# aponte411/minGPT-distributed

Measured on AMD Instinct MI355X. Metric: tokens/sec (whole node), GPT-2 124M seq1024 bf16, higher is better.
Workload: dtype bf16; 1 GPU; model=gpt2, global_batch=128, seq_len=1024, parallelism=dp1, micro_batch_per_gpu=128, hip_graph=False

## Files before the change

csrc/bindings.cpp:

```cpp
#include <torch/extension.h>
#include <ATen/hip/impl/HIPGuardImplMasqueradingAsCUDA.h>
#include <ATen/hip/impl/HIPStreamMasqueradingAsCUDA.h>

#include "comm.h"
#include "kernels.h"

namespace {

using mg::bf16_t;

hipStream_t cur_stream() { return c10::hip::getCurrentHIPStreamMasqueradingAsCUDA().stream(); }
using DevGuard = c10::hip::HIPGuardMasqueradingAsCUDA;

#define CHECK_DEV(t) TORCH_CHECK((t).is_cuda(), #t " must be a GPU tensor")
#define CHECK_CONTIG(t) TORCH_CHECK((t).is_contiguous(), #t " must be contiguous")
#define CHECK_BF16(t) \
  CHECK_DEV(t);       \
  TORCH_CHECK((t).scalar_type() == at::kBFloat16, #t " must be bf16")
#define CHECK_F32(t) \
  CHECK_DEV(t);      \
  TORCH_CHECK((t).scalar_type() == at::kFloat, #t " must be fp32")
#define CHECK_I64(t) \
  CHECK_DEV(t);      \
  TORCH_CHECK((t).scalar_type() == at::kLong, #t " must be int64")
// ... 82 lines not shown
  }
  const unsigned long long* ap = nullptr;
  int groups = 0;
  int64_t* seqp = nullptr;
  long seq_ld = 0;
  if (am_part.has_value()) {
    TORCH_CHECK(pd && am_part->scalar_type() == at::kLong && am_part->is_contiguous() && am_part->dim() == 2 &&
                am_part->size(0) == B, "embedding_fwd: am_part int64 [B, G] with pos_dev");
    ap = reinterpret_cast<const unsigned long long*>(am_part->data_ptr<int64_t>());
    groups = (int)am_part->size(1);
    if (seq.has_value()) {
      TORCH_CHECK(seq->scalar_type() == at::kLong && seq->is_contiguous() && seq->dim() == 2 && seq->size(0) == B,
                  "embedding_fwd: seq int64 [B, L]");
      seqp = seq->data_ptr<int64_t>();
      seq_ld = seq->size(1);
    }
  }
  DevGuard g(idx.device());
  auto out = at::empty({B, T, D}, wte.options());
  mg::embedding_fwd(idx.data_ptr<int64_t>(), bp(wte), bp(wpe), bp(out), (int)(B * T), (int)T,
                    (int)D, (int)wte.size(0), (float)p, (uint64_t)seed, cur_stream(), pd, ap, groups,
                    ap ? idx.data_ptr<int64_t>() : nullptr, seqp, seq_ld, (int)pos_stride, (int)wpe.size(0));
  return out;
}

void embedding_bwd(const at::Tensor& idx, const at::Tensor& dout,
                   const c10::optional<at::Tensor>& dwte, const c10::optional<at::Tensor>& dwpe,
                   double p, int64_t seed) {
  CHECK_I64(idx); CHECK_BF16(dout); CHECK_CONTIG(dout); CHECK_CONTIG(idx);
  const int64_t B = idx.size(0), T = idx.size(1), D = dout.size(-1);
  TORCH_CHECK(dout.numel() == B * T * D, "embedding_bwd: shape mismatch");
  if (dwte.has_value()) { CHECK_F32(*dwte); TORCH_CHECK(dwte->size(-1) == D); }
  if (dwpe.has_value()) { CHECK_F32(*dwpe); TORCH_CHECK(dwpe->size(-1) == D && dwpe->size(0) >= T); }
  DevGuard g(idx.device());
  mg::embedding_bwd(idx.data_ptr<int64_t>(), bp(dout), fp_opt(dwte), fp_opt(dwpe), (int)(B * T),
                    (int)T, (int)D, dwte.has_value() ? (int)(dwte->numel() / D) : 0, (float)p, (uint64_t)seed, cur_stream());
}

std::vector<at::Tensor> xent_fwd(const at::Tensor& logits, const at::Tensor& targets, int64_t V) {
  CHECK_BF16(logits); CHECK_I64(targets); CHECK_CONTIG(logits); CHECK_CONTIG(targets);
  const int64_t ld = logits.size(-1), M = logits.numel() / ld;
  TORCH_CHECK(targets.numel() == M && V <= ld && ld % 8 == 0, "xent: shape mismatch");
  DevGuard g(logits.device());
  auto opts = logits.options().dtype(at::kFloat);
  auto loss_row = at::empty({M}, opts);
  auto lse = at::empty({M}, opts);
  auto out = at::empty({2}, opts);
  mg::xent_fwd(bp(logits), targets.data_ptr<int64_t>(), fp(loss_row), fp(lse), fp(out), (int)M,
               (int)V, (int)ld, cur_stream());
  return {out, lse};
}

at::Tensor xent_bwd(const at::Tensor& logits, const at::Tensor& targets, const at::Tensor& lse,
                    const at::Tensor& gscale, const at::Tensor& out, int64_t V) {
  CHECK_BF16(logits); CHECK_I64(targets); CHECK_F32(lse); CHECK_F32(gscale); CHECK_F32(out);
  const int64_t ld = logits.size(-1), M = logits.numel() / ld;
  TORCH_CHECK(targets.numel() == M && lse.numel() == M, "xent_bwd: shape mismatch");
  DevGuard g(logits.device());
  auto dl = at::empty_like(logits);
  mg::xent_bwd(bp(logits), targets.data_ptr<int64_t>(), fp(lse), fp(gscale), fp(out) + 1, bp(dl),
               (int)M, (int)V, (int)ld, cur_stream());
  return dl;
}

std::vector<at::Tensor> xent_fused(const at::Tensor& logits, const at::Tensor& targets, int64_t V) {
  CHECK_BF16(logits); CHECK_I64(targets); CHECK_CONTIG(logits); CHECK_CONTIG(targets);
  const int64_t ld = logits.size(-1), M = logits.numel() / ld;
  TORCH_CHECK(targets.numel() == M && V <= ld && ld % 8 == 0, "xent_fused: shape mismatch");
  if (mg::xent_fused_nv((int)ld) == 0) return {};
  DevGuard g(logits.device());
  auto opts = logits.options().dtype(at::kFloat);
  auto loss_row = at::empty({M}, opts);
  auto out = at::empty({2}, opts);
  auto dl = at::empty_like(logits);
  mg::xent_fused(bp(logits), targets.data_ptr<int64_t>(), fp(loss_row), fp(out), bp(dl), (int)M,
                 (int)V, (int)ld, cur_stream());
  return {out, dl};
}

void xent_scale_(const at::Tensor& dlogits, const at::Tensor& gscale) {
  CHECK_BF16(dlogits); CHECK_CONTIG(dlogits); CHECK_F32(gscale);
  TORCH_CHECK(dlogits.numel() % 8 == 0, "xent_scale_: numel must be a multiple of 8");
  DevGuard g(dlogits.device());
  mg::xent_scale(bp(dlogits), fp(gscale), dlogits.numel(), cur_stream());
}

void set_graph_state(const c10::optional<at::Tensor>& seed_ofs, const c10::optional<at::Tensor>& opt_hp) {
  if (seed_ofs.has_value()) {
    TORCH_CHECK(seed_ofs->scalar_type() == at::kLong && seed_ofs->is_cuda() && seed_ofs->numel() >= 1);
  }
  if (opt_hp.has_value()) { CHECK_F32(*opt_hp); TORCH_CHECK(opt_hp->numel() >= 2); }
  mg::set_graph_state(seed_ofs.has_value() ? reinterpret_cast<const uint64_t*>(seed_ofs->data_ptr<int64_t>()) : nullptr,
                      opt_hp.has_value() ? fp(*opt_hp) : nullptr);
}

void grad_sumsq(const at::Tensor& grad, double grad_scale, const at::Tensor& out) {
  CHECK_F32(grad); CHECK_F32(out); CHECK_CONTIG(grad);
  TORCH_CHECK(out.numel() >= 2);
  DevGuard g(grad.device());
  auto ws = at::empty({(int64_t)(mg::grad_norm_workspace() / 4)}, grad.options());
  mg::grad_sumsq(fp(grad), grad.numel(), (float)grad_scale, fp(ws), fp(out), cur_stream());
}

void grad_sumsq_chunks(const at::Tensor& chunk_start, const at::Tensor& chunk_len,
                       const at::Tensor& grad, double grad_scale, const at::Tensor& out,
                       int64_t table_end) {
  CHECK_I64(chunk_start); CHECK_DEV(chunk_len); CHECK_CONTIG(grad); CHECK_F32(out);
  TORCH_CHECK(chunk_len.scalar_type() == at::kInt, "chunk_len must be int32");
// ... 112 lines not shown
at::Tensor transpose(const at::Tensor& src, int64_t ldd) {
  CHECK_BF16(src); CHECK_CONTIG(src);
  TORCH_CHECK(src.dim() == 2, "transpose: 2-D input");
  const int64_t R = src.size(0), C = src.size(1);
  if (ldd <= 0) ldd = R;
  TORCH_CHECK(ldd >= R, "transpose: ldd < rows");
  DevGuard g(src.device());
  auto dst = at::empty({C, ldd}, src.options());
  mg::transpose(bp(src), bp(dst), (int)R, (int)C, (int)ldd, cur_stream());
  return dst;
}

at::Tensor dropout_bwd(const at::Tensor& dy, double p, int64_t seed) {
  CHECK_BF16(dy); CHECK_CONTIG(dy);
  const int64_t N = dy.size(-1), M = dy.numel() / N;
  TORCH_CHECK(N % 8 == 0, "dropout_bwd: last dim must be a multiple of 8");
  DevGuard g(dy.device());
  auto dx = at::empty_like(dy);
  mg::dropout_bwd(bp(dy), bp(dx), M, (int)N, (float)p, (uint64_t)seed, cur_stream());
  return dx;
}

at::Tensor dropout_bias_grad(const at::Tensor& dy, const at::Tensor& db, double p, int64_t seed) {
  CHECK_BF16(dy); CHECK_F32(db); CHECK_CONTIG(dy);
  const int64_t N = dy.size(-1), M = dy.numel() / N;
  TORCH_CHECK(N % 8 == 0 && db.numel() == N, "dropout_bias_grad: shape mismatch");
  DevGuard g(dy.device());
  auto dx = at::empty_like(dy);
  mg::dropout_bias_grad(bp(dy), bp(dx), fp(db), M, (int)N, (float)p, (uint64_t)seed, cur_stream());
  return dx;
}

void bias_grad(const at::Tensor& dy, const at::Tensor& db) {
  CHECK_BF16(dy); CHECK_F32(db); CHECK_CONTIG(dy);
  const int64_t N = dy.size(-1), M = dy.numel() / N;
  TORCH_CHECK(N % 8 == 0 && db.numel() == N, "bias_grad: shape mismatch");
  DevGuard g(dy.device());
  mg::bias_grad(bp(dy), fp(db), M, (int)N, cur_stream());
}

void gemm(const at::Tensor& a, const at::Tensor& b, const at::Tensor& c, int64_t layout, int64_t epi,
          const c10::optional<at::Tensor>& bias, const c10::optional<at::Tensor>& aux,
          const c10::optional<at::Tensor>& resid, double p, int64_t seed, int64_t M, int64_t N,
          const c10::optional<at::Tensor>& dbias) {
  CHECK_BF16(a); CHECK_BF16(b); CHECK_DEV(c);
  CHECK_CONTIG(a); CHECK_CONTIG(b); CHECK_CONTIG(c);
  TORCH_CHECK(a.dim() == 2 && b.dim() == 2 && c.dim() == 2, "gemm: 2-D operands required");
  TORCH_CHECK(layout >= 0 && layout <= 2 && epi >= 0 && epi <= 7 && epi != 5, "gemm: bad layout/epilogue");
  TORCH_CHECK((epi != 6 || layout == 0) && (epi != 7 || layout == 1), "gemm: fragment-ordered GELU' epilogues: 6 NT, 7 NN");
  const int64_t lda = a.size(1), ldb = b.size(1), ldc = c.size(1);
  TORCH_CHECK(lda % 8 == 0 && ldb % 8 == 0 && ldc % 8 == 0, "gemm: row strides must be multiples of 8");
  TORCH_CHECK(M > 0 && N > 0 && M <= c.size(0) && N <= ldc, "gemm: output bounds");
  int64_t K, a_ext, b_ext, ka, kb;
  if (layout == 0) {
    K = lda; ka = lda; kb = ldb; a_ext = a.size(0); b_ext = b.size(0);
    TORCH_CHECK(lda == ldb, "gemm NT: K mismatch");
    TORCH_CHECK(M <= a_ext && N <= (epi == 0 ? ldc : b_ext), "gemm NT: shape mismatch");
    TORCH_CHECK(c.scalar_type() == at::kBFloat16, "gemm NT: bf16 output");
  } else if (layout == 1) {
    K = lda; ka = lda; kb = b.size(0); a_ext = a.size(0); b_ext = ldb;
    TORCH_CHECK(kb <= K && M <= a_ext && N <= ldb && (epi == 0 || epi == 4 || epi == 7), "gemm NN: shape mismatch");
    TORCH_CHECK(c.scalar_type() == at::kBFloat16, "gemm NN: bf16 output");
  } else {
    K = a.size(0); ka = K; kb = b.size(0); a_ext = lda; b_ext = ldb;
    TORCH_CHECK(kb == K && M <= lda && N <= ldb && epi == 0, "gemm TN: shape mismatch");
    TORCH_CHECK(c.scalar_type() == at::kFloat, "gemm TN: fp32 accumulate output");
  }
  TORCH_CHECK(K % 8 == 0, "gemm: K must be a multiple of 8");
  const bf16_t* bias_p = nullptr;
  if (bias.has_value() && bias->defined()) {
    CHECK_BF16(*bias);
// ... 720 lines not shown
```

csrc/include/kernels.h:

```cpp
#pragma once
#include <hip/hip_runtime.h>
#include <stddef.h>
#include <stdint.h>

namespace mg {
typedef uint16_t bf16_t;

void layernorm_fwd(const bf16_t* x, const bf16_t* w, const bf16_t* b, bf16_t* y, float* mean,
                   float* rstd, int M, int D, float eps, hipStream_t stream);
void layernorm_bwd(const bf16_t* dy, const bf16_t* x, const bf16_t* w, const float* mean,
                   const float* rstd, const bf16_t* dres, bf16_t* dx, float* dw, float* db,
                   float* workspace, int M, int D, hipStream_t stream, bf16_t* dz = nullptr,
                   float* dzb = nullptr, float p = 0.f, uint64_t seed = 0);
size_t layernorm_bwd_workspace(int M, int D, bool drop);
int ln_bwd_grid(int M, int D, bool drop);

void embedding_fwd(const int64_t* idx, const bf16_t* wte, const bf16_t* wpe, bf16_t* out, int M,
                   int T, int D, int V, float p, uint64_t seed, hipStream_t stream,
                   const int* pos_dev = nullptr,
                   const unsigned long long* am_part = nullptr,
                   int am_groups = 0,
                   int64_t* tok = nullptr,
                   int64_t* seq = nullptr,
                   long seq_ld = 0,
                   int pos_stride = 0,
                   int pos_rows = 0);
unsigned int debug_error_bits();
void embedding_bwd(const int64_t* idx, const bf16_t* dout, float* dwte, float* dwpe, int M, int T,
                   int D, int V, float p, uint64_t seed, hipStream_t stream);

void xent_fwd(const bf16_t* logits, const int64_t* targets, float* loss_row, float* lse, float* out,
              int M, int V, int ld, hipStream_t stream);
void xent_bwd(const bf16_t* logits, const int64_t* targets, const float* lse, const float* gscale,
              const float* inv_n, bf16_t* dlogits, int M, int V, int ld, hipStream_t stream);
int xent_fused_nv(int ld);
void xent_fused(const bf16_t* logits, const int64_t* targets, float* loss_row, float* out,
                bf16_t* dlogits, int M, int V, int ld, hipStream_t stream);
void xent_scale(bf16_t* dlogits, const float* gscale, long n, hipStream_t stream);

void set_graph_state(const uint64_t* seed_ofs, const float* opt_hp);
const uint64_t* graph_seed_ofs();
const float* graph_opt_hp();
size_t grad_norm_workspace();
void grad_sumsq(const float* grad, long n, float grad_scale, float* workspace, float* out,
                hipStream_t stream);
void grad_sumsq_chunks(const int64_t* chunk_start, const int* chunk_len, int n_chunks,
                       const void* grad, bool grad_bf16, float grad_scale, float* workspace,
                       float* out, hipStream_t stream);
void adamw_step(const int64_t* chunk_start, const int* chunk_len, const float* chunk_wd,
                const int64_t* moment_start, int n_chunks, float* master, bf16_t* param,
                const void* grad, bool grad_bf16, float* m, float* v, const float* norm, float lr,
                float b1, float b2, float eps, int step, float grad_scale, float clip,
                hipStream_t stream, float* zero_grad = nullptr);
void f32_to_bf16(const float* src, bf16_t* dst, long n, hipStream_t stream);
void comm_proxy(const void* src, void* dst, long n16, long total16, int channels, double gbps,
                hipStream_t stream);

constexpr int kGemvSegK = 4096;
bool gemv_supported(int B, int K);
struct GemvArgmax {
  unsigned long long* part;
  int* pos;
};
int gemv_grid(int N, int B);
void gemv(const bf16_t* x, const bf16_t* W, bf16_t* y, int B, int N, int K, long ldy, const bf16_t* bias,
          const bf16_t* resid, int epi, hipStream_t stream, const bf16_t* lnw = nullptr,
          const bf16_t* lnb = nullptr, float eps = 1e-5f, const GemvArgmax* am = nullptr);
bool gemv_nt_weights();
bool gemv_w8_supported(int B, int K);
// ... 86 lines not shown
```

csrc/kernels/elementwise.hip:

```cpp
#include "common.h"
#include "kernels.h"

using namespace mg;

namespace {

constexpr int kGrid = 4096;

__global__ __launch_bounds__(256) void bias_act_kernel(const bf16_t* __restrict__ x,
                                                       const bf16_t* __restrict__ b,
                                                       bf16_t* __restrict__ pre,
                                                       bf16_t* __restrict__ y, long n8, int N,
                                                       int act) {
  for (long i = (long)blockIdx.x * 256 + threadIdx.x; i < n8; i += (long)gridDim.x * 256) {
    const long e = i * 8;
    const int c = (int)(e % N);
    float v[8], bb[8];
    unpack8(ld16(x + e), v);
    if (b) {
      unpack8(ld16(b + c), bb);
#pragma unroll
      for (int j = 0; j < 8; ++j) v[j] += bb[j];
    }
    if (act == 1) {
// ... 65 lines not shown
                                                                bf16_t* __restrict__ dx,
                                                                float* __restrict__ db, int M, int N,
                                                                uint64_t seed, uint32_t thr,
                                                                float scale, const uint64_t* sofs) {
  constexpr int RG = 256 / CVB;
  __shared__ __attribute__((aligned(16))) float red[RG][CVB * 8];
  seed = eff_seed(seed, sofs);
  const int cv = threadIdx.x % CVB, rg = threadIdx.x / CVB;
  const int c = (blockIdx.x * CVB + cv) * 8;
  float s[8] = {0, 0, 0, 0, 0, 0, 0, 0};
  if (c < N) {
    for (long r = (long)blockIdx.y * RG + rg; r < M; r += (long)gridDim.y * RG) {
      float g[8];
      const long e = r * N + c;
      unpack8(ld16(dy + e), g);
      rowdrop8(g, seed, r, c, N, thr, scale);
      st16(dx + e, pack8(g));
#pragma unroll
      for (int j = 0; j < 8; ++j) s[j] += g[j];
    }
  }
#pragma unroll
  for (int j = 0; j < 8; ++j) red[rg][cv * 8 + j] = s[j];
  __syncthreads();
  for (int k = threadIdx.x; k < CVB * 8; k += 256) {
    const int col = blockIdx.x * CVB * 8 + k;
    float t = 0.f;
#pragma unroll
    for (int i = 0; i < RG; ++i) t += red[i][k];
    if (col < N) atomicAdd(db + col, t);
  }
}

template <int CVB>
__global__ __launch_bounds__(256) void bias_grad_kernel(const bf16_t* __restrict__ dy,
                                                        float* __restrict__ db, int M, int N, long ld) {
  constexpr int RG = 256 / CVB;
  __shared__ __attribute__((aligned(16))) float red[RG][CVB * 8];
  const int cv = threadIdx.x % CVB, rg = threadIdx.x / CVB;
  const int c = (blockIdx.x * CVB + cv) * 8;
  float s[8] = {0, 0, 0, 0, 0, 0, 0, 0};
  if (c < N) {
    for (long r = (long)blockIdx.y * RG + rg; r < M; r += (long)gridDim.y * RG) {
      float g[8];
      unpack8(ld16(dy + r * ld + c), g);
#pragma unroll
      for (int j = 0; j < 8; ++j) s[j] += g[j];
    }
  }
#pragma unroll
  for (int j = 0; j < 8; ++j) red[rg][cv * 8 + j] = s[j];
  __syncthreads();
  for (int k = threadIdx.x; k < CVB * 8; k += 256) {
    const int col = blockIdx.x * CVB * 8 + k;
    float t = 0.f;
#pragma unroll
    for (int i = 0; i < RG; ++i) t += red[i][k];
    if (col < N) atomicAdd(db + col, t);
  }
}

__global__ __launch_bounds__(256) void transpose_kernel(const bf16_t* __restrict__ src,
                                                        bf16_t* __restrict__ dst, int R, int C,
                                                        int ldd) {
  __shared__ uint4 t[16 * 8 * 16];
  const int r0 = blockIdx.y * 128, c0 = blockIdx.x * 128;
  {
    const int rb = threadIdx.x >> 4, cb = threadIdx.x & 15;
    uint32_t w[8][4];
#pragma unroll
    for (int i = 0; i < 8; ++i) {
      const int r = r0 + 8 * rb + i, c = c0 + 8 * cb;
      uint4 v = make_uint4(0, 0, 0, 0);
      if (r < R) {
        if (c + 8 <= C) {
          v = ld16(src + (long)r * C + c);
        } else if (c < C) {
          alignas(16) bf16_t e[8] = {0, 0, 0, 0, 0, 0, 0, 0};
          for (int q = 0; q < 8 && c + q < C; ++q) e[q] = src[(long)r * C + c + q];
          v = *reinterpret_cast<const uint4*>(e);
// ... 61 lines not shown
                                                       graph_seed_ofs());
}

static int bias_cvb(int N) { return ((N / 8) % 64 != 0 && (N / 8) % 32 == 0) ? 32 : 64; }

static dim3 bias_grid(long M, int N, int cvb) {
  const int cx = cdiv(N, cvb * 8);
  int ry = (int)std::max<long>(1, std::min<long>(512, M / 64));
  while (cx * ry > 2048 && ry > 1) ry >>= 1;
  return dim3(cx, ry);
}

void dropout_bias_grad(const bf16_t* dy, bf16_t* dx, float* db, long M, int N, float p, uint64_t seed,
                       hipStream_t stream) {
  const uint32_t thr = dropout_threshold16(p);
  const int cvb = bias_cvb(N);
  const dim3 grid = bias_grid(M, N, cvb);
  if (cvb == 32)
    dropout_bias_grad_kernel<32><<<grid, 256, 0, stream>>>(dy, dx, db, (int)M, N, seed, thr,
                                                           dropout_scale16(thr), graph_seed_ofs());
  else
    dropout_bias_grad_kernel<64><<<grid, 256, 0, stream>>>(dy, dx, db, (int)M, N, seed, thr,
                                                           dropout_scale16(thr), graph_seed_ofs());
}

void transpose(const bf16_t* src, bf16_t* dst, int R, int C, int ldd, hipStream_t stream) {
  transpose_kernel<<<dim3(cdiv(C, 128), cdiv(ldd, 128)), 256, 0, stream>>>(src, dst, R, C, ldd);
}

void bias_grad(const bf16_t* dy, float* db, long M, int N, hipStream_t stream, long ld) {
  const int cvb = bias_cvb(N);
  const dim3 grid = bias_grid(M, N, cvb);
  if (ld <= 0) ld = N;
  if (cvb == 32)
    bias_grad_kernel<32><<<grid, 256, 0, stream>>>(dy, db, (int)M, N, ld);
  else
    bias_grad_kernel<64><<<grid, 256, 0, stream>>>(dy, db, (int)M, N, ld);
}

}
```

csrc/kernels/embedding.hip:

```cpp
#include "common.h"
#include "kernels.h"

using namespace mg;

namespace {

__global__ __launch_bounds__(256) void emb_fwd_kernel(const int64_t* __restrict__ idx,
                                                      const bf16_t* __restrict__ wte,
                                                      const bf16_t* __restrict__ wpe,
                                                      bf16_t* __restrict__ out, int M, int T, int D, int V,
                                                      unsigned int* __restrict__ err,
                                                      uint64_t seed, uint32_t thr, float scale,
                                                      int use_dropout, const uint64_t* sofs,
                                                      const int* __restrict__ pos_dev, int pos_stride,
                                                      int pos_rows,
                                                      const unsigned long long* __restrict__ am_part,
                                                      int am_groups, int64_t* __restrict__ tok_out,
                                                      int64_t* __restrict__ seq, long seq_ld) {
  const int lane = threadIdx.x & 63;
  const long m = (long)blockIdx.x * 4 + (threadIdx.x >> 6);
  if (m >= M) return;
  seed = eff_seed(seed, sofs);
  long tok;
  if (am_part) {
    unsigned long long best = 0;
    for (int i = lane; i < am_groups; i += 64) {
      const unsigned long long k = am_part[m * am_groups + i];
      best = k > best ? k : best;
    }
#pragma unroll
    for (int o = 32; o > 0; o >>= 1) {
      const unsigned lo = __shfl_xor((unsigned)best, o, 64), hi = __shfl_xor((unsigned)(best >> 32), o, 64);
      const unsigned long long k = ((unsigned long long)hi << 32) | lo;
      best = k > best ? k : best;
    }
    tok = amax_index(best);
    if (lane == 0) {
      if (tok_out) tok_out[m] = tok;
      if (seq) seq[m * seq_ld + *pos_dev] = tok;
    }
  } else {
    tok = idx[m];
  }
  MG_CHECK_INDEX(tok, tok >= 0 && tok < V, 0, err, 1u)
  int t = pos_dev ? *pos_dev : (int)(m % T);
  if (pos_dev && pos_stride) t = min(max(pos_dev[m * pos_stride], 0), pos_rows - 1);
  for (int c = lane * 8; c < D; c += 512) {
    float a[8], p[8];
    unpack8(ld16(wte + tok * D + c), a);
    unpack8(ld16(wpe + (long)t * D + c), p);
#pragma unroll
    for (int j = 0; j < 8; ++j) a[j] += p[j];
    if (use_dropout) rowdrop8(a, seed, m, c, D, thr, scale);
    st16(out + m * D + c, pack8(a));
  }
}

__global__ __launch_bounds__(256) void emb_bwd_wte_kernel(const int64_t* __restrict__ idx,
                                                          const bf16_t* __restrict__ dout,
                                                          float* __restrict__ dwte, int M, int D, int V,
                                                          unsigned int* __restrict__ err,
                                                          uint64_t seed, uint32_t thr, float scale,
                                                          int use_dropout, const uint64_t* sofs) {
  const int lane = threadIdx.x & 63;
  const long m = (long)blockIdx.x * 4 + (threadIdx.x >> 6);
  if (m >= M) return;
  seed = eff_seed(seed, sofs);
  long tok = idx[m];
  MG_CHECK_INDEX(tok, tok >= 0 && tok < V, 0, err, 2u)
  for (int c0 = 0; c0 < D; c0 += 512) {
    const int c = c0 + lane * 8;
    float g[8];
    if (c < D) {
      unpack8(ld16(dout + m * D + c), g);
      if (use_dropout) rowdrop8(g, seed, m, c, D, thr, scale);
    }
#pragma unroll
    for (int k = 0; k < 8; ++k) {
      const int src = 8 * k + (lane >> 3);
      float val = 0.f;
#pragma unroll
      for (int j = 0; j < 8; ++j) {
        const float t = __shfl(g[j], src, 64);
        if ((lane & 7) == j) val = t;
      }
      const int col = c0 + 64 * k + lane;
      if (col < D) atomicAdd(dwte + tok * D + col, val);
    }
  }
}

__global__ __launch_bounds__(64) void emb_bwd_wpe_kernel(const bf16_t* __restrict__ dout,
                                                         float* __restrict__ dwpe, int B, int T, int D,
                                                         uint64_t seed, uint32_t thr, float scale,
                                                         int use_dropout, const uint64_t* sofs) {
  const int t = blockIdx.x;
  const int c = blockIdx.y * 512 + threadIdx.x * 8;
  if (c >= D) return;
  seed = eff_seed(seed, sofs);
  float s[8] = {0, 0, 0, 0, 0, 0, 0, 0};
  for (int b = 0; b < B; ++b) {
    const long m = (long)b * T + t;
    float g[8];
    unpack8(ld16(dout + m * D + c), g);
    if (use_dropout) rowdrop8(g, seed, m, c, D, thr, scale);
#pragma unroll
    for (int j = 0; j < 8; ++j) s[j] += g[j];
  }
  float* dst = dwpe + (long)t * D + c;
#pragma unroll
  for (int j = 0; j < 8; ++j) dst[j] += s[j];
}

}

namespace mg {

void embedding_fwd(const int64_t* idx, const bf16_t* wte, const bf16_t* wpe, bf16_t* out, int M,
                   int T, int D, int V, float p, uint64_t seed, hipStream_t stream, const int* pos_dev,
                   const unsigned long long* am_part, int am_groups, int64_t* tok, int64_t* seq,
                   long seq_ld, int pos_stride, int pos_rows) {
  const uint32_t thr = dropout_threshold16(p);
  emb_fwd_kernel<<<cdiv(M, 4), 256, 0, stream>>>(idx, wte, wpe, out, M, T, D, V, debug_err_word(), seed, thr,
                                                 dropout_scale16(thr), p > 0.f,
                                                 graph_seed_ofs(), pos_dev, pos_stride, pos_rows, am_part,
                                                 am_groups, tok, seq, seq_ld);
}

void embedding_bwd(const int64_t* idx, const bf16_t* dout, float* dwte, float* dwpe, int M, int T,
                   int D, int V, float p, uint64_t seed, hipStream_t stream) {
  const uint32_t thr = dropout_threshold16(p);
  const float scale = dropout_scale16(thr);
  if (dwte)
    emb_bwd_wte_kernel<<<cdiv(M, 4), 256, 0, stream>>>(idx, dout, dwte, M, D, V, debug_err_word(), seed, thr, scale,
                                                       p > 0.f, graph_seed_ofs());
  if (dwpe) {
    dim3 grid(T, cdiv(D, 512));
    emb_bwd_wpe_kernel<<<grid, 64, 0, stream>>>(dout, dwpe, M / T, T, D, seed, thr, scale, p > 0.f,
                                                graph_seed_ofs());
  }
}

unsigned int* debug_err_word() {
#ifdef MG_DEBUG
  static unsigned int* w = nullptr;
  if (!w) {
    (void)hipMalloc(&w, sizeof(unsigned int));
    (void)hipMemset(w, 0, sizeof(unsigned int));
  }
  return w;
#else
  return nullptr;
#endif
}

unsigned int debug_error_bits() {
#ifdef MG_DEBUG
  unsigned int v = 0u;
  (void)hipDeviceSynchronize();
  (void)hipMemcpy(&v, debug_err_word(), sizeof(v), hipMemcpyDeviceToHost);
  (void)hipMemset(debug_err_word(), 0, sizeof(v));
  (void)hipDeviceSynchronize();
  return v;
#else
  return 0u;
#endif
}

}
```

csrc/kernels/xent.hip:

```cpp
#include "common.h"
#include "kernels.h"

using namespace mg;

namespace {

__global__ __launch_bounds__(256) void xent_fwd_kernel(const bf16_t* __restrict__ logits,
                                                       const int64_t* __restrict__ targets,
                                                       float* __restrict__ loss_row,
                                                       float* __restrict__ lse_out, int V, int ld,
                                                       unsigned int* __restrict__ err) {
  __shared__ float red[8];
  const long row = blockIdx.x;
  const bf16_t* lr = logits + row * ld;
  float mx = -INFINITY, sm = 0.f;
  const int V8 = V & ~7;
  for (int c = threadIdx.x * 8; c < V8; c += 256 * 8) {
    float v[8];
    unpack8(ld16(lr + c), v);
    float lm = v[0];
#pragma unroll
    for (int j = 1; j < 8; ++j) lm = fmaxf(lm, v[j]);
    if (lm > mx) {
      sm *= __expf(mx - lm);
      mx = lm;
    }
#pragma unroll
    for (int j = 0; j < 8; ++j) sm += __expf(v[j] - mx);
  }
  for (int c = V8 + threadIdx.x; c < V; c += 256) {
    const float v = bf2f(lr[c]);
    if (v > mx) {
      sm *= __expf(mx - v);
      mx = v;
    }
    sm += __expf(v - mx);
  }
  const float gmx = block_max<4>(mx, red);
  sm = (mx == -INFINITY) ? 0.f : sm * __expf(mx - gmx);
  const float gsm = block_sum<4>(sm, red + 4);
  if (threadIdx.x == 0) {
    const float lse = gmx + __logf(gsm);
    lse_out[row] = lse;
    long t = targets[row];
  MG_CHECK_INDEX(t, t < V, -1, err, 4u)
    loss_row[row] = (t < 0) ? 0.f : lse - bf2f(lr[t]);
  }
}

__global__ __launch_bounds__(1024) void xent_finalize_kernel(const float* __restrict__ loss_row,
                                                             const int64_t* __restrict__ targets,
                                                             float* __restrict__ out, int M) {
  __shared__ float red[32];
  float s = 0.f, n = 0.f;
  for (int i = threadIdx.x; i < M; i += 1024) {
    s += loss_row[i];
    n += targets[i] >= 0 ? 1.f : 0.f;
  }
  s = block_sum<16>(s, red);
  n = block_sum<16>(n, red + 16);
  if (threadIdx.x == 0) {
    const float inv = n > 0.f ? 1.f / n : 0.f;
    out[0] = s * inv;
    out[1] = inv;
  }
}

__global__ __launch_bounds__(256) void xent_bwd_kernel(const bf16_t* __restrict__ logits,
                                                       const int64_t* __restrict__ targets,
                                                       const float* __restrict__ lse,
                                                       const float* __restrict__ gscale,
                                                       const float* __restrict__ inv_n,
                                                       bf16_t* __restrict__ dlogits, int V, int ld,
                                                       unsigned int* __restrict__ err) {
  const long row = blockIdx.x;
  long t = targets[row];
  MG_CHECK_INDEX(t, t < V, -1, err, 4u)
  const float g = (t < 0) ? 0.f : gscale[0] * inv_n[0];
  const float l = lse[row];
  const bf16_t* lr = logits + row * ld;
  bf16_t* dr = dlogits + row * ld;
  for (int c = threadIdx.x * 8; c < ld; c += 256 * 8) {
    float v[8];
    if (c + 8 <= V) {
      unpack8(ld16(lr + c), v);
#pragma unroll
      for (int j = 0; j < 8; ++j) v[j] = g * (__expf(v[j] - l) - ((c + j) == t ? 1.f : 0.f));
    } else {
#pragma unroll
      for (int j = 0; j < 8; ++j) {
        const int cj = c + j;
        v[j] = cj < V ? g * (__expf(bf2f(lr[cj]) - l) - (cj == t ? 1.f : 0.f)) : 0.f;
      }
    }
    st16(dr + c, pack8(v));
  }
}


__global__ __launch_bounds__(1024) void xent_count_kernel(const int64_t* __restrict__ targets,
                                                          float* __restrict__ out, int M) {
  __shared__ float red[16];
  float n = 0.f;
  for (int i = threadIdx.x; i < M; i += 1024) n += targets[i] >= 0 ? 1.f : 0.f;
  n = block_sum<16>(n, red);
  if (threadIdx.x == 0) out[1] = n > 0.f ? 1.f / n : 0.f;
}

template <int NV>
__global__ __launch_bounds__(1024) void xent_fused_kernel(const bf16_t* __restrict__ logits,
                                                          const int64_t* __restrict__ targets,
                                                          const float* __restrict__ inv_n,
                                                          float* __restrict__ loss_row,
                                                          bf16_t* __restrict__ dlogits, int V,
                                                          int ld, unsigned int* __restrict__ err) {
  __shared__ float red[32];
  const long row = blockIdx.x;
  const bf16_t* lr = logits + row * ld;
  bf16_t* dr = dlogits + row * ld;
  constexpr uint32_t NEG2 = 0xFF80FF80u;
  uint4 u[NV];
#pragma unroll
  for (int k = 0; k < NV; ++k) {
    const int c = (threadIdx.x + k * 1024) * 8;
    if (c + 8 <= V) {
      u[k] = ld16_nt(lr + c);
    } else if (c < V) {
      float f[8];
#pragma unroll
      for (int j = 0; j < 8; ++j) f[j] = (c + j < V) ? bf2f(lr[c + j]) : -INFINITY;
      u[k] = pack8(f);
    } else {
      u[k] = make_uint4(NEG2, NEG2, NEG2, NEG2);
    }
  }
  float mx = -INFINITY;
#pragma unroll
  for (int k = 0; k < NV; ++k) {
    float v[8];
    unpack8(u[k], v);
#pragma unroll
    for (int j = 0; j < 8; ++j) mx = fmaxf(mx, v[j]);
  }
  const float gmx = block_max<16>(mx, red);
#pragma unroll
  for (int k = 0; k < NV; ++k) reg_fence(u[k]);
  constexpr float L2E = 1.4426950408889634f;
  const float mb = gmx * L2E;
  float sm = 0.f;
#pragma unroll
  for (int k = 0; k < NV; ++k) {
    float v[8];
    unpack8(u[k], v);
#pragma unroll
    for (int j = 0; j < 8; ++j) sm += exp2f(fmaf(v[j], L2E, -mb));
  }
  const float gsm = block_sum<16>(sm, red + 16);
#pragma unroll
  for (int k = 0; k < NV; ++k) reg_fence(u[k]);
  const float lse = gmx + __logf(gsm);
  long t = targets[row];
  MG_CHECK_INDEX(t, t < V, -1, err, 4u)
  const float g = (t < 0) ? 0.f : inv_n[0];
  const float lb = lse * L2E;
#pragma unroll
  for (int k = 0; k < NV; ++k) {
    const int c = (threadIdx.x + k * 1024) * 8;
    if (c < ld) {
      float v[8];
      unpack8(u[k], v);
#pragma unroll
      for (int j = 0; j < 8; ++j) v[j] = g * (exp2f(fmaf(v[j], L2E, -lb)) - ((c + j) == t ? 1.f : 0.f));
      st16_nt(dr + c, pack8(v));
    }
  }
  if (threadIdx.x == 0) loss_row[row] = (t < 0) ? 0.f : lse - bf2f(lr[t]);
}

__global__ __launch_bounds__(256) void xent_scale_kernel(bf16_t* __restrict__ dl,
                                                         const float* __restrict__ gscale, long n8) {
  const float s = gscale[0];
  if (s == 1.f) return;
  for (long i = blockIdx.x * 256L + threadIdx.x; i < n8; i += (long)gridDim.x * 256) {
    float v[8];
    unpack8(ld16(dl + i * 8), v);
#pragma unroll
    for (int j = 0; j < 8; ++j) v[j] *= s;
    st16(dl + i * 8, pack8(v));
  }
}

}

namespace mg {

void xent_fwd(const bf16_t* logits, const int64_t* targets, float* loss_row, float* lse, float* out,
              int M, int V, int ld, hipStream_t stream) {
  xent_fwd_kernel<<<M, 256, 0, stream>>>(logits, targets, loss_row, lse, V, ld, debug_err_word());
  xent_finalize_kernel<<<1, 1024, 0, stream>>>(loss_row, targets, out, M);
}

void xent_bwd(const bf16_t* logits, const int64_t* targets, const float* lse, const float* gscale,
              const float* inv_n, bf16_t* dlogits, int M, int V, int ld, hipStream_t stream) {
  xent_bwd_kernel<<<M, 256, 0, stream>>>(logits, targets, lse, gscale, inv_n, dlogits, V, ld, debug_err_word());
}

}

namespace mg {

int xent_fused_nv(int ld) {
  const int nv = (ld / 8 + 1023) / 1024;
  return (nv >= 4 && nv <= 8) ? nv : 0;
}

void xent_fused(const bf16_t* logits, const int64_t* targets, float* loss_row, float* out,
                bf16_t* dlogits, int M, int V, int ld, hipStream_t stream) {
  xent_count_kernel<<<1, 1024, 0, stream>>>(targets, out, M);
  switch (xent_fused_nv(ld)) {
#define MG_XF(n) \
  case n: xent_fused_kernel<n><<<M, 1024, 0, stream>>>(logits, targets, out + 1, loss_row, dlogits, V, ld, debug_err_word()); break;
    MG_XF(4) MG_XF(5) MG_XF(6) MG_XF(7) MG_XF(8)
#undef MG_XF
    default: break;
  }
  xent_finalize_kernel<<<1, 1024, 0, stream>>>(loss_row, targets, out, M);
}

void xent_scale(bf16_t* dlogits, const float* gscale, long n, hipStream_t stream) {
  const long n8 = n / 8;
  const long blocks = std::min<long>((n8 + 255) / 256, 2048);
  xent_scale_kernel<<<(int)blocks, 256, 0, stream>>>(dlogits, gscale, n8);
}

}
```

Baseline: 1.147 million tokens/s.

## Sort tokens for embedding backward, parallelize xent reductions, unroll bias grad

Embedding wte backward now builds a token histogram, prefix scan and sorted order, then accumulates runs of equal tokens in registers. This replaces one atomic per row element with far fewer atomics. The wpe backward uses four waves per block with a shared-memory reduction. The cross-entropy count and finalize steps become a multi-block partial reduction plus a one-wave finalize instead of single-block kernels, and bias_grad gains multi-row unrolled loads for strided column slices. The cost is extra kernel launches and a zeroed workspace allocation on each call.

```diff
diff --git a/csrc/bindings.cpp b/csrc/bindings.cpp
--- a/csrc/bindings.cpp
+++ b/csrc/bindings.cpp
@@ -138,9 +138,14 @@
   TORCH_CHECK(dout.numel() == B * T * D, "embedding_bwd: shape mismatch");
   if (dwte.has_value()) { CHECK_F32(*dwte); TORCH_CHECK(dwte->size(-1) == D); }
   if (dwpe.has_value()) { CHECK_F32(*dwpe); TORCH_CHECK(dwpe->size(-1) == D && dwpe->size(0) >= T); }
+  TORCH_CHECK(D % 8 == 0 && (!fp_opt(dwte) || (uintptr_t)fp_opt(dwte) % 16 == 0),
+              "embedding_bwd: D must be a multiple of 8 and dwte 16-byte aligned");
   DevGuard g(idx.device());
-  mg::embedding_bwd(idx.data_ptr<int64_t>(), bp(dout), fp_opt(dwte), fp_opt(dwpe), (int)(B * T),
-                    (int)T, (int)D, dwte.has_value() ? (int)(dwte->numel() / D) : 0, (float)p, (uint64_t)seed, cur_stream());
+  const int64_t V = fp_opt(dwte) ? dwte->numel() / D : 0;
+  at::Tensor ws;
+  if (fp_opt(dwte)) ws = at::zeros({mg::embedding_bwd_workspace((int)(B * T), (int)V)}, idx.options().dtype(at::kInt));
+  mg::embedding_bwd(idx.data_ptr<int64_t>(), bp(dout), fp_opt(dwte), fp_opt(dwpe), ws.defined() ? ws.data_ptr<int>() : nullptr,
+                    (int)(B * T), (int)T, (int)D, (int)V, (float)p, (uint64_t)seed, cur_stream());
 }
 
 std::vector<at::Tensor> xent_fwd(const at::Tensor& logits, const at::Tensor& targets, int64_t V) {
@@ -152,7 +157,8 @@
   auto loss_row = at::empty({M}, opts);
   auto lse = at::empty({M}, opts);
   auto out = at::empty({2}, opts);
-  mg::xent_fwd(bp(logits), targets.data_ptr<int64_t>(), fp(loss_row), fp(lse), fp(out), (int)M,
+  auto ws = at::empty({mg::xent_scalar_workspace()}, opts);
+  mg::xent_fwd(bp(logits), targets.data_ptr<int64_t>(), fp(loss_row), fp(lse), fp(out), fp(ws), (int)M,
                (int)V, (int)ld, cur_stream());
   return {out, lse};
 }
@@ -179,7 +185,8 @@
   auto loss_row = at::empty({M}, opts);
   auto out = at::empty({2}, opts);
   auto dl = at::empty_like(logits);
-  mg::xent_fused(bp(logits), targets.data_ptr<int64_t>(), fp(loss_row), fp(out), bp(dl), (int)M,
+  auto ws = at::empty({mg::xent_scalar_workspace()}, opts);
+  mg::xent_fused(bp(logits), targets.data_ptr<int64_t>(), fp(loss_row), fp(out), fp(ws), bp(dl), (int)M,
                  (int)V, (int)ld, cur_stream());
   return {out, dl};
 }
@@ -358,11 +365,19 @@
 }
 
 void bias_grad(const at::Tensor& dy, const at::Tensor& db) {
-  CHECK_BF16(dy); CHECK_F32(db); CHECK_CONTIG(dy);
+  CHECK_BF16(dy); CHECK_F32(db);
+  const bool slice = dy.dim() == 2 && !dy.is_contiguous();
+  if (slice) {
+    TORCH_CHECK(dy.stride(1) == 1 && dy.stride(0) >= dy.size(1) && dy.stride(0) % 8 == 0 &&
+                (uintptr_t)dy.data_ptr() % 16 == 0, "bias_grad: a column slice needs unit column stride, "
+                "a row stride that is a multiple of 8 and a 16-byte aligned start");
+  } else {
+    CHECK_CONTIG(dy);
+  }
   const int64_t N = dy.size(-1), M = dy.numel() / N;
-  TORCH_CHECK(N % 8 == 0 && db.numel() == N, "bias_grad: shape mismatch");
+  TORCH_CHECK(N % 8 == 0 && db.numel() == N && db.is_contiguous(), "bias_grad: shape mismatch");
   DevGuard g(dy.device());
-  mg::bias_grad(bp(dy), fp(db), M, (int)N, cur_stream());
+  mg::bias_grad(bp(dy), fp(db), M, (int)N, cur_stream(), slice ? dy.stride(0) : 0);
 }
 
 void gemm(const at::Tensor& a, const at::Tensor& b, const at::Tensor& c, int64_t layout, int64_t epi,
diff --git a/csrc/include/kernels.h b/csrc/include/kernels.h
--- a/csrc/include/kernels.h
+++ b/csrc/include/kernels.h
@@ -26,15 +26,17 @@
                    int pos_stride = 0,
                    int pos_rows = 0);
 unsigned int debug_error_bits();
-void embedding_bwd(const int64_t* idx, const bf16_t* dout, float* dwte, float* dwpe, int M, int T,
+long embedding_bwd_workspace(int M, int V);
+void embedding_bwd(const int64_t* idx, const bf16_t* dout, float* dwte, float* dwpe, int* ws, int M, int T,
                    int D, int V, float p, uint64_t seed, hipStream_t stream);
 
+long xent_scalar_workspace();
 void xent_fwd(const bf16_t* logits, const int64_t* targets, float* loss_row, float* lse, float* out,
-              int M, int V, int ld, hipStream_t stream);
+              float* ws, int M, int V, int ld, hipStream_t stream);
 void xent_bwd(const bf16_t* logits, const int64_t* targets, const float* lse, const float* gscale,
               const float* inv_n, bf16_t* dlogits, int M, int V, int ld, hipStream_t stream);
 int xent_fused_nv(int ld);
-void xent_fused(const bf16_t* logits, const int64_t* targets, float* loss_row, float* out,
+void xent_fused(const bf16_t* logits, const int64_t* targets, float* loss_row, float* out, float* ws,
                 bf16_t* dlogits, int M, int V, int ld, hipStream_t stream);
 void xent_scale(bf16_t* dlogits, const float* gscale, long n, hipStream_t stream);
 
diff --git a/csrc/kernels/elementwise.hip b/csrc/kernels/elementwise.hip
--- a/csrc/kernels/elementwise.hip
+++ b/csrc/kernels/elementwise.hip
@@ -121,7 +121,9 @@
   }
 }
 
-template <int CVB>
+constexpr int kBiasRows = 4;
+
+template <int CVB, int ROWS>
 __global__ __launch_bounds__(256) void bias_grad_kernel(const bf16_t* __restrict__ dy,
                                                         float* __restrict__ db, int M, int N, long ld) {
   constexpr int RG = 256 / CVB;
@@ -130,11 +132,33 @@
   const int c = (blockIdx.x * CVB + cv) * 8;
   float s[8] = {0, 0, 0, 0, 0, 0, 0, 0};
   if (c < N) {
-    for (long r = (long)blockIdx.y * RG + rg; r < M; r += (long)gridDim.y * RG) {
-      float g[8];
-      unpack8(ld16(dy + r * ld + c), g);
-#pragma unroll
-      for (int j = 0; j < 8; ++j) s[j] += g[j];
+    float a[ROWS][8] = {};
+    const long step = (long)gridDim.y * RG;
+    for (long r = (long)blockIdx.y * RG + rg; r < M; r += ROWS * step) {
+      uint4 u[ROWS];
+#pragma unroll
+      for (int i = 0; i < ROWS; ++i) {
+        const long ri = r + i * step;
+        u[i] = ri < M ? ld16(dy + ri * ld + c) : make_uint4(0, 0, 0, 0);
+      }
+#pragma unroll
+      for (int i = 0; i < ROWS; ++i) {
+        float g[8];
+        unpack8(u[i], g);
+#pragma unroll
+        for (int j = 0; j < 8; ++j) a[i][j] += g[j];
+      }
+    }
+#pragma unroll
+    for (int j = 0; j < 8; ++j) {
+      float h[ROWS];
+#pragma unroll
+      for (int i = 0; i < ROWS; ++i) h[i] = a[i][j];
+#pragma unroll
+      for (int w = ROWS / 2; w > 0; w >>= 1)
+#pragma unroll
+        for (int i = 0; i < w; ++i) h[i] += h[i + w];
+      s[j] = h[0];
     }
   }
 #pragma unroll
@@ -262,10 +286,16 @@
   const int cvb = bias_cvb(N);
   const dim3 grid = bias_grid(M, N, cvb);
   if (ld <= 0) ld = N;
-  if (cvb == 32)
-    bias_grad_kernel<32><<<grid, 256, 0, stream>>>(dy, db, (int)M, N, ld);
-  else
-    bias_grad_kernel<64><<<grid, 256, 0, stream>>>(dy, db, (int)M, N, ld);
-}
-
-}
+  if (ld > N) {
+    if (cvb == 32)
+      bias_grad_kernel<32, kBiasRows><<<grid, 256, 0, stream>>>(dy, db, (int)M, N, ld);
+    else
+      bias_grad_kernel<64, kBiasRows><<<grid, 256, 0, stream>>>(dy, db, (int)M, N, ld);
+  } else if (cvb == 32) {
+    bias_grad_kernel<32, 1><<<grid, 256, 0, stream>>>(dy, db, (int)M, N, ld);
+  } else {
+    bias_grad_kernel<64, 1><<<grid, 256, 0, stream>>>(dy, db, (int)M, N, ld);
+  }
+}
+
+}
diff --git a/csrc/kernels/embedding.hip b/csrc/kernels/embedding.hip
--- a/csrc/kernels/embedding.hip
+++ b/csrc/kernels/embedding.hip
@@ -56,60 +56,219 @@
   }
 }
 
+
+constexpr int kCH = 32;
+
+MG_DEVICE void emb_wave_groups(int tok, bool valid, int lane, int& leader, int& rank, int& size) {
+  unsigned long long todo = __ballot(valid);
+  leader = lane, rank = 0, size = 0;
+  while (todo) {
+    const int l = __ffsll((long long)todo) - 1;
+    const int t = __shfl(tok, l, 64);
+    const unsigned long long same = __ballot(valid && tok == t);
+    if (valid && tok == t) {
+      leader = l;
+      rank = __popcll(same & ((1ull << lane) - 1ull));
+      size = __popcll(same);
+    }
+    todo &= ~same;
+  }
+}
+
+MG_DEVICE bool emb_token(const int64_t* __restrict__ idx, int m, int M, int V, unsigned int* err, int& tok) {
+  if (m >= M) return false;
+  long t = idx[m];
+  MG_CHECK_INDEX(t, t >= 0 && t < V, 0, err, 2u)
+  tok = (int)t;
+  return t >= 0 && t < V;
+}
+
+__global__ __launch_bounds__(256) void emb_hist_kernel(const int64_t* __restrict__ idx, int* __restrict__ cnt,
+                                                       int M, int V, unsigned int* __restrict__ err) {
+  int tok = 0, leader, rank, size;
+  const bool valid = emb_token(idx, blockIdx.x * 256 + threadIdx.x, M, V, err, tok);
+  emb_wave_groups(tok, valid, threadIdx.x & 63, leader, rank, size);
+  if (valid && rank == 0) atomicAdd(cnt + tok, size);
+}
+
+__global__ __launch_bounds__(1024) void emb_scan_kernel(int* __restrict__ cnt, int* __restrict__ total, int Vp) {
+  __shared__ int wsum[2][16];
+  const int lane = threadIdx.x & 63, w = threadIdx.x >> 6;
+  const int tiles = (Vp + 4095) / 4096;
+  const int4 zero = make_int4(0, 0, 0, 0);
+  int4* c4 = reinterpret_cast<int4*>(cnt);
+  int carry = 0;
+  int4 nxt = (int)threadIdx.x * 4 < Vp ? c4[threadIdx.x] : zero;
+  for (int k = 0; k < tiles; ++k) {
+    const int i4 = k * 1024 + threadIdx.x;
+    const int4 v = nxt;
+    nxt = (i4 + 1024) * 4 < Vp ? c4[i4 + 1024] : zero;
+    const int s = v.x + v.y + v.z + v.w;
+    int inc = s;
+#pragma unroll
+    for (int o = 1; o < 64; o <<= 1) {
+      const int t = __shfl_up(inc, o, 64);
+      if (lane >= o) inc += t;
+    }
+    if (lane == 63) wsum[k & 1][w] = inc;
+    __syncthreads();
+    int base = carry + inc - s, tot = 0;
+#pragma unroll
+    for (int i = 0; i < 16; ++i) {
+      const int t = wsum[k & 1][i];
+      if (i < w) base += t;
+      tot += t;
+    }
+    carry += tot;
+    if (i4 * 4 < Vp) c4[i4] = make_int4(base, base + v.x, base + v.x + v.y, base + v.x + v.y + v.z);
+  }
+  if (threadIdx.x == 0) *total = carry;
+}
+
+__global__ __launch_bounds__(256) void emb_fill_kernel(const int64_t* __restrict__ idx, int* __restrict__ cur,
+                                                       int* __restrict__ order, int M, int V,
+                                                       unsigned int* __restrict__ err) {
+  const int m = blockIdx.x * 256 + threadIdx.x;
+  int tok = 0, leader, rank, size;
+  const bool valid = emb_token(idx, m, M, V, err, tok);
+  emb_wave_groups(tok, valid, threadIdx.x & 63, leader, rank, size);
+  int slot = 0;
+  if (valid && rank == 0) slot = atomicAdd(cur + tok, size);
+  slot = __shfl(slot, leader, 64);
+  if (valid) order[slot + rank] = m;
+}
+
+MG_DEVICE void emb_flush(float* __restrict__ row, int c0, int lane, int D, const float (&s)[8], bool alone) {
+  if (alone) {
+    const int c = c0 + lane * 8;
+    if (c < D) {
+      float4* p = reinterpret_cast<float4*>(row + c);
+      float4 a = p[0], b = p[1];
+      a.x += s[0]; a.y += s[1]; a.z += s[2]; a.w += s[3];
+      b.x += s[4]; b.y += s[5]; b.z += s[6]; b.w += s[7];
+      p[0] = a;
+      p[1] = b;
+    }
+    return;
+  }
+#pragma unroll
+  for (int k = 0; k < 8; ++k) {
+    const int src = 8 * k + (lane >> 3);
+    float val = 0.f;
+#pragma unroll
+    for (int j = 0; j < 8; ++j) {
+      const float t = __shfl(s[j], src, 64);
+      if ((lane & 7) == j) val = t;
+    }
+    const int col = c0 + 64 * k + lane;
+    if (col < D) atomicAdd(row + col, val);
+  }
+}
+
+template <int CH>
 __global__ __launch_bounds__(256) void emb_bwd_wte_kernel(const int64_t* __restrict__ idx,
+                                                          const int* __restrict__ order,
+                                                          const int* __restrict__ total,
                                                           const bf16_t* __restrict__ dout,
-                                                          float* __restrict__ dwte, int M, int D, int V,
+                                                          float* __restrict__ dwte, int D, int V,
                                                           unsigned int* __restrict__ err,
                                                           uint64_t seed, uint32_t thr, float scale,
                                                           int use_dropout, const uint64_t* sofs) {
+  static_assert(CH % 4 == 0 && CH <= 32, "one lane per sorted row and two for its neighbours, walked four at a time");
   const int lane = threadIdx.x & 63;
-  const long m = (long)blockIdx.x * 4 + (threadIdx.x >> 6);
-  if (m >= M) return;
+  const int n = *total;
+  const long lo = ((long)blockIdx.x * 4 + __builtin_amdgcn_readfirstlane(threadIdx.x >> 6)) * CH;
+  if (lo >= n) return;
+  const int cnt = (int)min((long)CH, n - lo);
   seed = eff_seed(seed, sofs);
-  long tok = idx[m];
-  MG_CHECK_INDEX(tok, tok >= 0 && tok < V, 0, err, 2u)
+  long pos = lo + lane;
+  if (lane == CH) pos = lo - 1;
+  if (lane == CH + 1) pos = lo + cnt;
+  int m_l = 0, t_l = -1;
+  if ((lane < cnt || lane == CH || lane == CH + 1) && pos >= 0 && pos < n) {
+    m_l = order[pos];
+    emb_token(idx, m_l, INT_MAX, V, err, t_l);
+  }
+  const int tprev = __builtin_amdgcn_readlane(t_l, CH), tnext = __builtin_amdgcn_readlane(t_l, CH + 1);
   for (int c0 = 0; c0 < D; c0 += 512) {
     const int c = c0 + lane * 8;
-    float g[8];
-    if (c < D) {
-      unpack8(ld16(dout + m * D + c), g);
-      if (use_dropout) rowdrop8(g, seed, m, c, D, thr, scale);
-    }
-#pragma unroll
-    for (int k = 0; k < 8; ++k) {
-      const int src = 8 * k + (lane >> 3);
-      float val = 0.f;
-#pragma unroll
-      for (int j = 0; j < 8; ++j) {
-        const float t = __shfl(g[j], src, 64);
-        if ((lane & 7) == j) val = t;
+    float s[8] = {0, 0, 0, 0, 0, 0, 0, 0};
+    int tok = __builtin_amdgcn_readfirstlane(t_l);
+    bool alone = tok != tprev;
+    for (int i0 = 0; i0 < cnt; i0 += 4) {
+      uint4 u[4];
+      int mj[4], tj[4];
+#pragma unroll
+      for (int j = 0; j < 4; ++j) {
+        const int i = min(i0 + j, cnt - 1);
+        mj[j] = __builtin_amdgcn_readlane(m_l, i);
+        tj[j] = __builtin_amdgcn_readlane(t_l, i);
+        u[j] = make_uint4(0, 0, 0, 0);
+        if (c < D && i0 + j < cnt) u[j] = ld16(dout + (long)mj[j] * D + c);
       }
-      const int col = c0 + 64 * k + lane;
-      if (col < D) atomicAdd(dwte + tok * D + col, val);
-    }
-  }
-}
-
-__global__ __launch_bounds__(64) void emb_bwd_wpe_kernel(const bf16_t* __restrict__ dout,
-                                                         float* __restrict__ dwpe, int B, int T, int D,
-                                                         uint64_t seed, uint32_t thr, float scale,
-                                                         int use_dropout, const uint64_t* sofs) {
+#pragma unroll
+      for (int j = 0; j < 4; ++j) {
+        if (i0 + j >= cnt) break;
+        if (tj[j] != tok) {
+          emb_flush(dwte + (long)tok * D, c0, lane, D, s, alone);
+#pragma unroll
+          for (int q = 0; q < 8; ++q) s[q] = 0.f;
+          tok = tj[j];
+          alone = true;
+        }
+        float g[8];
+        unpack8(u[j], g);
+        if (use_dropout && c < D) rowdrop8(g, seed, mj[j], c, D, thr, scale);
+#pragma unroll
+        for (int q = 0; q < 8; ++q) s[q] += g[q];
+      }
+    }
+    emb_flush(dwte + (long)tok * D, c0, lane, D, s, alone && tok != tnext);
+  }
+}
+
+__global__ __launch_bounds__(256) void emb_bwd_wpe_kernel(const bf16_t* __restrict__ dout,
+                                                          float* __restrict__ dwpe, int B, int T, int D,
+                                                          uint64_t seed, uint32_t thr, float scale,
+                                                          int use_dropout, const uint64_t* sofs) {
+  __shared__ float red[3][8][64];
+  const int lane = threadIdx.x & 63, w = threadIdx.x >> 6;
   const int t = blockIdx.x;
-  const int c = blockIdx.y * 512 + threadIdx.x * 8;
-  if (c >= D) return;
+  const int c = blockIdx.y * 512 + lane * 8;
+  const bool on = c < D;
   seed = eff_seed(seed, sofs);
   float s[8] = {0, 0, 0, 0, 0, 0, 0, 0};
-  for (int b = 0; b < B; ++b) {
-    const long m = (long)b * T + t;
-    float g[8];
-    unpack8(ld16(dout + m * D + c), g);
-    if (use_dropout) rowdrop8(g, seed, m, c, D, thr, scale);
-#pragma unroll
-    for (int j = 0; j < 8; ++j) s[j] += g[j];
-  }
-  float* dst = dwpe + (long)t * D + c;
-#pragma unroll
-  for (int j = 0; j < 8; ++j) dst[j] += s[j];
+  const int b0 = (int)((long)B * w / 4), b1 = (int)((long)B * (w + 1) / 4);
+  if (on) {
+    for (int b = b0; b < b1; b += 4) {
+      uint4 u[4];
+#pragma unroll
+      for (int j = 0; j < 4; ++j) {
+        const long m = (long)min(b + j, b1 - 1) * T + t;
+        u[j] = ld16(dout + m * D + c);
+      }
+#pragma unroll
+      for (int j = 0; j < 4; ++j) {
+        if (b + j >= b1) break;
+        const long m = (long)(b + j) * T + t;
+        float g[8];
+        unpack8(u[j], g);
+        if (use_dropout) rowdrop8(g, seed, m, c, D, thr, scale);
+#pragma unroll
+        for (int q = 0; q < 8; ++q) s[q] += g[q];
+      }
+    }
+  }
+  if (w > 0) {
+#pragma unroll
+    for (int q = 0; q < 8; ++q) red[w - 1][q][lane] = s[q];
+  }
+  __syncthreads();
+  if (w == 0 && on) {
+    float* dst = dwpe + (long)t * D + c;
+#pragma unroll
+    for (int q = 0; q < 8; ++q) dst[q] += ((s[q] + red[0][q][lane]) + red[1][q][lane]) + red[2][q][lane];
+  }
 }
 
 }
@@ -127,17 +286,27 @@
                                                  am_groups, tok, seq, seq_ld);
 }
 
-void embedding_bwd(const int64_t* idx, const bf16_t* dout, float* dwte, float* dwpe, int M, int T,
+static int emb_vp(int V) { return (V + 3) & ~3; }
+
+long embedding_bwd_workspace(int M, int V) { return (long)emb_vp(V) + 4 + M; }
+
+void embedding_bwd(const int64_t* idx, const bf16_t* dout, float* dwte, float* dwpe, int* ws, int M, int T,
                    int D, int V, float p, uint64_t seed, hipStream_t stream) {
   const uint32_t thr = dropout_threshold16(p);
   const float scale = dropout_scale16(thr);
-  if (dwte)
-    emb_bwd_wte_kernel<<<cdiv(M, 4), 256, 0, stream>>>(idx, dout, dwte, M, D, V, debug_err_word(), seed, thr, scale,
-                                                       p > 0.f, graph_seed_ofs());
+  if (dwte) {
+    int *cnt = ws, *total = ws + emb_vp(V), *order = total + 4;
+    emb_hist_kernel<<<cdiv(M, 256), 256, 0, stream>>>(idx, cnt, M, V, debug_err_word());
+    emb_scan_kernel<<<1, 1024, 0, stream>>>(cnt, total, emb_vp(V));
+    emb_fill_kernel<<<cdiv(M, 256), 256, 0, stream>>>(idx, cnt, order, M, V, debug_err_word());
+    emb_bwd_wte_kernel<kCH><<<cdiv(M, 4 * kCH), 256, 0, stream>>>(idx, order, total, dout, dwte, D, V,
+                                                                  debug_err_word(), seed, thr, scale, p > 0.f,
+                                                                  graph_seed_ofs());
+  }
   if (dwpe) {
     dim3 grid(T, cdiv(D, 512));
-    emb_bwd_wpe_kernel<<<grid, 64, 0, stream>>>(dout, dwpe, M / T, T, D, seed, thr, scale, p > 0.f,
-                                                graph_seed_ofs());
+    emb_bwd_wpe_kernel<<<grid, 256, 0, stream>>>(dout, dwpe, M / T, T, D, seed, thr, scale, p > 0.f,
+                                                 graph_seed_ofs());
   }
 }
 
diff --git a/csrc/kernels/xent.hip b/csrc/kernels/xent.hip
--- a/csrc/kernels/xent.hip
+++ b/csrc/kernels/xent.hip
@@ -48,17 +48,36 @@
   }
 }
 
-__global__ __launch_bounds__(1024) void xent_finalize_kernel(const float* __restrict__ loss_row,
-                                                             const int64_t* __restrict__ targets,
-                                                             float* __restrict__ out, int M) {
-  __shared__ float red[32];
+constexpr int kXG = 128;
+
+__global__ __launch_bounds__(256) void xent_partial_kernel(const float* __restrict__ loss_row,
+                                                           const int64_t* __restrict__ targets,
+                                                           float* __restrict__ part, int M) {
+  __shared__ float red[8];
+  const int per = (M + gridDim.x - 1) / gridDim.x;
+  const int lo = blockIdx.x * per, hi = min(lo + per, M);
   float s = 0.f, n = 0.f;
-  for (int i = threadIdx.x; i < M; i += 1024) {
-    s += loss_row[i];
+  for (int i = lo + threadIdx.x; i < hi; i += 256) {
+    if (loss_row) s += loss_row[i];
     n += targets[i] >= 0 ? 1.f : 0.f;
   }
-  s = block_sum<16>(s, red);
-  n = block_sum<16>(n, red + 16);
+  n = block_sum<4>(n, red);
+  s = block_sum<4>(s, red + 4);
+  if (threadIdx.x == 0) {
+    part[blockIdx.x] = n;
+    if (loss_row) part[kXG + blockIdx.x] = s;
+  }
+}
+
+MG_DEVICE float wave_partials(const float* __restrict__ part, int G, int lane) {
+  float v = lane < G ? part[lane] : 0.f;
+  if (lane + 64 < G) v += part[lane + 64];
+  return wave_sum(v);
+}
+
+__global__ __launch_bounds__(64) void xent_finalize_kernel(const float* __restrict__ part, int G,
+                                                           float* __restrict__ out) {
+  const float n = wave_partials(part, G, threadIdx.x), s = wave_partials(part + kXG, G, threadIdx.x);
   if (threadIdx.x == 0) {
     const float inv = n > 0.f ? 1.f / n : 0.f;
     out[0] = s * inv;
@@ -98,23 +117,14 @@
 }
 
 
-__global__ __launch_bounds__(1024) void xent_count_kernel(const int64_t* __restrict__ targets,
-                                                          float* __restrict__ out, int M) {
-  __shared__ float red[16];
-  float n = 0.f;
-  for (int i = threadIdx.x; i < M; i += 1024) n += targets[i] >= 0 ? 1.f : 0.f;
-  n = block_sum<16>(n, red);
-  if (threadIdx.x == 0) out[1] = n > 0.f ? 1.f / n : 0.f;
-}
-
 template <int NV>
 __global__ __launch_bounds__(1024) void xent_fused_kernel(const bf16_t* __restrict__ logits,
                                                           const int64_t* __restrict__ targets,
-                                                          const float* __restrict__ inv_n,
+                                                          const float* __restrict__ cnt_part, int G,
                                                           float* __restrict__ loss_row,
                                                           bf16_t* __restrict__ dlogits, int V,
                                                           int ld, unsigned int* __restrict__ err) {
-  __shared__ float red[32];
+  __shared__ float red[33];
   const long row = blockIdx.x;
   const bf16_t* lr = logits + row * ld;
   bf16_t* dr = dlogits + row * ld;
@@ -134,6 +144,10 @@
       u[k] = make_uint4(NEG2, NEG2, NEG2, NEG2);
     }
   }
+  if (threadIdx.x < 64) {
+    const float n = wave_partials(cnt_part, G, threadIdx.x);
+    if (threadIdx.x == 0) red[32] = n > 0.f ? 1.f / n : 0.f;
+  }
   float mx = -INFINITY;
 #pragma unroll
   for (int k = 0; k < NV; ++k) {
@@ -161,7 +175,7 @@
   const float lse = gmx + __logf(gsm);
   long t = targets[row];
   MG_CHECK_INDEX(t, t < V, -1, err, 4u)
-  const float g = (t < 0) ? 0.f : inv_n[0];
+  const float g = (t < 0) ? 0.f : red[32];
   const float lb = lse * L2E;
 #pragma unroll
   for (int k = 0; k < NV; ++k) {
@@ -194,10 +208,21 @@
 
 namespace mg {
 
+long xent_scalar_workspace() { return 3 * kXG; }
+
+static int xent_groups(int M) { return std::max(1, std::min(kXG, cdiv(M, 1024))); }
+
+static void xent_finalize(const float* loss_row, const int64_t* targets, float* out, float* ws, int M,
+                          hipStream_t stream) {
+  const int G = xent_groups(M);
+  xent_partial_kernel<<<G, 256, 0, stream>>>(loss_row, targets, ws + kXG, M);
+  xent_finalize_kernel<<<1, 64, 0, stream>>>(ws + kXG, G, out);
+}
+
 void xent_fwd(const bf16_t* logits, const int64_t* targets, float* loss_row, float* lse, float* out,
-              int M, int V, int ld, hipStream_t stream) {
+              float* ws, int M, int V, int ld, hipStream_t stream) {
   xent_fwd_kernel<<<M, 256, 0, stream>>>(logits, targets, loss_row, lse, V, ld, debug_err_word());
-  xent_finalize_kernel<<<1, 1024, 0, stream>>>(loss_row, targets, out, M);
+  xent_finalize(loss_row, targets, out, ws, M, stream);
 }
 
 void xent_bwd(const bf16_t* logits, const int64_t* targets, const float* lse, const float* gscale,
@@ -214,17 +239,18 @@
   return (nv >= 4 && nv <= 8) ? nv : 0;
 }
 
-void xent_fused(const bf16_t* logits, const int64_t* targets, float* loss_row, float* out,
+void xent_fused(const bf16_t* logits, const int64_t* targets, float* loss_row, float* out, float* ws,
                 bf16_t* dlogits, int M, int V, int ld, hipStream_t stream) {
-  xent_count_kernel<<<1, 1024, 0, stream>>>(targets, out, M);
+  const int G = xent_groups(M);
+  xent_partial_kernel<<<G, 256, 0, stream>>>(nullptr, targets, ws, M);
   switch (xent_fused_nv(ld)) {
 #define MG_XF(n) \
-  case n: xent_fused_kernel<n><<<M, 1024, 0, stream>>>(logits, targets, out + 1, loss_row, dlogits, V, ld, debug_err_word()); break;
+  case n: xent_fused_kernel<n><<<M, 1024, 0, stream>>>(logits, targets, ws, G, loss_row, dlogits, V, ld, debug_err_word()); break;
     MG_XF(4) MG_XF(5) MG_XF(6) MG_XF(7) MG_XF(8)
 #undef MG_XF
     default: break;
   }
-  xent_finalize_kernel<<<1, 1024, 0, stream>>>(loss_row, targets, out, M);
+  xent_finalize(loss_row, targets, out, ws, M, stream);
 }
 
 void xent_scale(bf16_t* dlogits, const float* gscale, long n, hipStream_t stream) {
```

Measured after the change: 1.149 million tokens/s, median of 6. No clear change (+0.2%).
